# jmackey-astro/PION

Measured on AMD Instinct MI355X. Metric: Mcell-updates/s on 3D ideal-MHD 512³ uniform grid; achieved HBM GB/s vs peak, higher is better.
Workload: dtype f64; 1 GPU; M1: 3-D GLM-MHD (nvar 9) Stone blast wave 512^3, HLLD + FKJ98 eta 0.1, periodic, OA2/OA2; nvar=9, decomposition=z-slab x1, transport=none; time loop and transport issued from C++ (libpion_host), fp_mode=fast (FMA contraction)

## Files before the change

pion_amd/csrc/kernels.h:

```cpp
#ifndef PION_KERNELS_H
#define PION_KERNELS_H

#include <hip/hip_runtime.h>
#include <stdint.h>

#include "dev_riemann.h"
#include "grid_desc.h"
#include "rows_tiling.h"
#include "hll_screen.h"

namespace pion {

#define PION_MAX_NTR 2
#define PION_COOL_NT_MAX 256

struct CoolDev {
  int NT;
  const double *T;
  const double *tab;
  const double *slope;
  double inv_Mu2, inv_Mu2_elec_H, Mu_tot_over_kB;
  double MinT_allowed, MaxT_allowed;
  float lg0, inv_dlg;
};
// ... 27 lines not shown
  static constexpr int lds = 11 * PION_COOL_NT_MAX;
};

struct StageArgs {
  GridDesc g;
  const double *S;
  const double *Pc;
  double *out;
  const uint8_t *flags;
  const uint8_t *hllflag;
  const double *eta;
  int *errword;
  FluxCtx fc;
  int eqntype, ntracer, solver;
  int space_ooa;
  int cooling;
  double dt;
  double glm_damp;
  double max_temp;
  int use_march;
  int xwrap;
  int zslope_lds;
  double *dE;
  int zchunk;
  int nzb, zcmax;
  int rows;
  int rows_auto;
  int ncu;
  int kz0, kz1;
  int kz2, kz3;
  unsigned long long *dtres;
  double cfl;
  int dt_mp;
  int plain_cells;
  CoolDev cool;
  unsigned long long *hsum;
  long hsum_n;
  int hsum_nbx, hsum_nby, hsum_nbz;
};

struct PrepassArgs {
  GridDesc g;
  const double *S;
  uint8_t *hllflag;
  double *divv, *gradp;
  double *eta;
  int eqntype, nvar, space_ooa;
  double gamma;
  long c0, c1;
  long c2, c3;
  const unsigned long long *hsum;
  ScrGeom scr;
  int *scr_list, *scr_count;
};

struct DtArgs {
  GridDesc g;
  const double *P;
  const double *Ph;
  const uint8_t *flags;
  unsigned long long *result;
  int *errword;
  int eqntype, nvar;
  double gamma, cfl;
  int do_mp;
  CoolDev cool;
};

struct FluxTestArgs {
  int n, axis, eqntype, ntracer, solver;
  const double *Pl, *Pr, *aux;
  double *F, *Pstar;
  int *errword;
  FluxCtx fc;
};

struct CellTestArgs {
  int n, eqntype, ntracer;
  const double *Pin, *dU;
  double *Pout, *dt;
  StageArgs st;
};

struct CoolTestArgs {
  int n, nvar;
  double dt, gamma;
  const double *Pin;
  double *Pout;
  const double *rho, *T;
  double *edot;
  int *errword;
  CoolDev cool;
};

#define PION_PER_EQN(FN, ARGS, ...)                                            \
  int FN##_hd(const ARGS &a, __VA_OPT__(__VA_ARGS__ x, ) hipStream_t s);       \
  int FN##_mhd(const ARGS &a, __VA_OPT__(__VA_ARGS__ x, ) hipStream_t s);      \
  int FN##_glm(const ARGS &a, __VA_OPT__(__VA_ARGS__ x, ) hipStream_t s);      \
  inline int FN(const ARGS &a, __VA_OPT__(__VA_ARGS__ x, ) hipStream_t s)      \
  {                                                                            \
    if (a.eqntype == EQEUL) return FN##_hd(a, __VA_OPT__(x, ) s);              \
    if (a.eqntype == EQMHD) return FN##_mhd(a, __VA_OPT__(x, ) s);             \
    if (a.eqntype == EQGLM) return FN##_glm(a, __VA_OPT__(x, ) s);             \
    return -1;                                                                 \
  }

#define PION_DECLARE_FP(NS)                                        \
// ... 18 lines not shown
```

pion_amd/csrc/kernels_prepass.hip:

```cpp
#include "dev_cooling.h"
#include "kernels.h"

#ifndef PION_FPNS
#error "PION_FPNS must be defined (fp_strict or fp_fast)"
#endif

namespace pion {
namespace PION_FPNS {

#include "dev_sweep.h"

PDEV void prepass_hlld_cell(const PrepassArgs &a, const int *i);

__global__ __launch_bounds__(256) void k_prepass_hlld(const PrepassArgs a)
{
  const long nc = a.g.ncell;
  const unsigned gx = (a.g.nga[0] + 63) / 64, gy = (a.g.nga[1] + 3) / 4;
  const long plane = (long)a.g.nga[0] * a.g.nga[1];
  const unsigned npl1 = (unsigned)((a.c1 - a.c0) / plane);
  const unsigned npl = npl1 + ((a.c3 > a.c2) ? (unsigned)((a.c3 - a.c2) / plane) : 0u);
  const unsigned ntile = gx * gy * npl;
  const unsigned t = (unsigned)xcd_tile(blockIdx.x, ntile);
  if (t >= ntile) return;
  int i[3];
// ... 153 lines not shown
        if (s >= nvs) {
          eL[s] = eR[s] = 0.0;
          continue;
        }
        const double *b = a.S + (long)(mhd ? rotvar<true>(ax, s) : rotvar<false>(ax, s)) * nc + c;
        const double q0 = b[0], q1 = b[st];
        double s0 = 0.0, s1 = 0.0;
        if (oa2 && a.g.cyl == 2) {
          const double R0 = sph_R(a.g, k), R1 = sph_R(a.g, k + 1);
          const double c0 = sph_Rcom(R0, dx), c1 = sph_Rcom(R1, dx);
          if (k > 0) s0 = avg_falle((q0 - b[-st]) / (c0 - sph_Rcom(sph_R(a.g, k - 1), dx)), (q1 - q0) / (c1 - c0));
          if (k + 1 < n - 1) s1 = avg_falle((q1 - q0) / (c1 - c0), (b[2 * st] - q1) / (sph_Rcom(sph_R(a.g, k + 2), dx) - c1));
          eL[s] = q0 + s0 * (R0 + 0.5 * dx - c0);
          eR[s] = q1 + s1 * (R1 - 0.5 * dx - c1);
        }
        else if (oa2 && a.g.cyl == 1 && ax == 1) {
          const double R0 = cyl_R(a.g, k), R1 = cyl_R(a.g, k + 1);
          const double c0 = cyl_Rcom(R0, dx), c1 = cyl_Rcom(R1, dx);
          if (k > 0) s0 = avg_falle((q0 - b[-st]) / (c0 - cyl_Rcom(cyl_R(a.g, k - 1), dx)), (q1 - q0) / (c1 - c0));
          if (k + 1 < n - 1) s1 = avg_falle((q1 - q0) / (c1 - c0), (b[2 * st] - q1) / (cyl_Rcom(cyl_R(a.g, k + 2), dx) - c1));
          eL[s] = q0 + s0 * (R0 + dx * 0.5 - c0);
          eR[s] = q1 + s1 * (R1 - dx * 0.5 - c1);
        }
        else if (oa2) {
          if (k > 0) s0 = avg_falle((q0 - b[-st]) / dx, (q1 - q0) / dx);
          if (k + 1 < n - 1) s1 = avg_falle((q1 - q0) / dx, (b[2 * st] - q1) / dx);
          eL[s] = q0 + s0 * dx * 0.5;
          eR[s] = q1 - s1 * dx * 0.5;
        }
        else {
          eL[s] = q0;
          eR[s] = q1;
        }
      }
      double msL, msR;
      if (mhd) {
        msL = Eqn<EQMHD, 0>::cfast(eL, g);
        msR = Eqn<EQMHD, 0>::cfast(eR, g);
      }
      else {
        msL = Eqn<EQEUL, 0>::chydro(eL, g);
        msR = Eqn<EQEUL, 0>::chydro(eR, g);
      }
      eta = 0.5 * (fabs(eR[qVN] - eL[qVN]) + fabs(msR - msL));
    }
    a.eta[ax * nc + c] = eta;
  }
}

__global__ __launch_bounds__(256) void k_prepass_screen(const PrepassArgs a)
{
  const long nblk = scr_total(a.scr);
  const long t = (long)blockIdx.x * blockDim.x + threadIdx.x;
  if (t >= nblk) return;
  const int bx = (int)(t % a.scr.nb[0]), by = (int)((t / a.scr.nb[0]) % a.scr.nb[1]);
  const int bz = (int)(t / ((long)a.scr.nb[0] * a.scr.nb[1]));
  if (!scr_block_quiet(a.scr, a.hsum, a.hsum + nblk, bx, by, bz)) a.scr_list[atomicAdd(a.scr_count, 1)] = (int)t;
}
__global__ __launch_bounds__(256) void k_prepass_hlld_blocks(const PrepassArgs a)
{
  const int n = *a.scr_count;
  for (int e = (int)blockIdx.x; e < n; e += (int)gridDim.x) {
    const int t = a.scr_list[e];
    const int bx = t % a.scr.nb[0], by = (t / a.scr.nb[0]) % a.scr.nb[1], bz = t / (a.scr.nb[0] * a.scr.nb[1]);
    int lo[3], hi[3];
    scr_cells_ext(a.scr, 0, bx, &lo[0], &hi[0]);
    scr_cells_ext(a.scr, 1, by, &lo[1], &hi[1]);
    scr_cells_ext(a.scr, 2, bz, &lo[2], &hi[2]);
    const int ny = hi[1] - lo[1], nrow = ny * (hi[2] - lo[2]);
    for (int r = (int)(threadIdx.x >> 6); r < nrow; r += 4) {
      int i[3];
      i[1] = lo[1] + r % ny;
      i[2] = lo[2] + r / ny;
      for (i[0] = lo[0] + (int)(threadIdx.x & 63); i[0] < hi[0]; i[0] += 64) prepass_hlld_cell(a, i);
    }
  }
}

int launch_prepass(const PrepassArgs &a, hipStream_t s)
{
  const unsigned nb = (unsigned)((a.c1 - a.c0 + 255) / 256);
  if (a.hllflag && a.hsum) {
    const long nblk = scr_total(a.scr);
    if (hipMemsetAsync(a.hllflag, 0, (size_t)a.g.ncell, s) != hipSuccess) return -1;
    if (hipMemsetAsync(a.scr_count, 0, sizeof(int), s) != hipSuccess) return -1;
    hipLaunchKernelGGL(k_prepass_screen, dim3((unsigned)((nblk + 255) / 256)), dim3(256), 0, s, a);
    const unsigned ngrid = (nblk < 4096) ? (unsigned)nblk : 4096u;
    hipLaunchKernelGGL(k_prepass_hlld_blocks, dim3(ngrid), dim3(256), 0, s, a);
  }
  else if (a.hllflag) {
    const long plane = (long)a.g.nga[0] * a.g.nga[1];
    const unsigned npl = (unsigned)((a.c1 - a.c0) / plane) + ((a.c3 > a.c2) ? (unsigned)((a.c3 - a.c2) / plane) : 0u);
    const unsigned ntile = (unsigned)((a.g.nga[0] + 63) / 64) * ((a.g.nga[1] + 3) / 4) * npl;
    if (a.g.ndim == 2 && (a.c0 != 0 || a.c1 != a.g.ncell)) {
      const long row = a.g.nga[0];
      const unsigned nr = (unsigned)((a.c1 - a.c0) / row) + ((a.c3 > a.c2) ? (unsigned)((a.c3 - a.c2) / row) : 0u);
      if (nr > 0)
        hipLaunchKernelGGL(k_prepass_hlld_rows, dim3((unsigned)((a.g.nga[0] + 63) / 64) * ((nr + 3) / 4)), dim3(256), 0,
                           s, a);
    }
    else if (a.g.ndim == 3 && a.g.cyl == 0 && !a.divv && !a.gradp && a.c3 <= a.c2 && npl >= PION_PREPASS_ZC
        && a.g.ncell * 8L < (1L << 32)) {
      const unsigned nch = (npl + PION_PREPASS_ZC - 1) / PION_PREPASS_ZC;
      const unsigned nt = (unsigned)((a.g.nga[0] + 61) / 62) * ((a.g.nga[1] + 3) / 4) * nch;
      hipLaunchKernelGGL(k_prepass_hlld_march, dim3(((nt + 7) / 8) * 8), dim3(256), 0, s, a);
    }
    else hipLaunchKernelGGL(k_prepass_hlld, dim3(((ntile + 7) / 8) * 8), dim3(256), 0, s, a);
  }
  if (a.eta) hipLaunchKernelGGL((k_prepass_hcorr<8>), dim3(nb), dim3(256), 0, s, a);
  return (int)hipGetLastError();
}

}
}
```

pion_amd/csrc/pion_gpu.hip:

```cpp
#include <hip/hip_runtime.h>

#include <cmath>
#include <cstdio>
#include <cstdlib>
#include <cstring>

#include "pion_handle.h"

using namespace pion;
using namespace pion::impl;

int impl::order_after_unpack(Handle *h)
{
  if (h->comm_stream && h->comm_stream != h->stream && h->ev_unpacked_valid) {
    HCHECK(h, hipStreamWaitEvent(h->stream, h->ev_unpacked, 0));
    h->ev_unpacked_valid = false;
  }
  return 0;
}

long impl::cell_id(const GridDesc &g, int ix, int iy, int iz)
{
  return (long)(ix + g.nbc[0]) + g.sy * (iy + g.nbc[1]) + g.sz * (iz + g.nbc[2]);
}
// ... 179 lines not shown
    if (hipDeviceGetAttribute(&ncu, hipDeviceAttributeMultiprocessorCount, device) == hipSuccess) h->ncu = ncu;
  }
  GridDesc &g = h->g;
  g.ndim = cfg->ndim;
  g.ncell = 1;
  for (int a = 0; a < 3; a++) {
    g.ng[a] = (a < cfg->ndim) ? cfg->ng[a] : 1;
    g.nbc[a] = (a < cfg->ndim) ? cfg->nbc : 0;
    g.nga[a] = g.ng[a] + 2 * g.nbc[a];
    g.ncell *= g.nga[a];
    g.xmin[a] = cfg->xmin[a];
  }
  g.sy = g.nga[0];
  g.sz = (long)g.nga[0] * g.nga[1];
  g.dx = cfg->dx;
  g.cyl = (cfg->coord_sys == 2) ? 1 : ((cfg->coord_sys == 3) ? 2 : 0);
  g.sph_vol = nullptr;
  *handle = h;
  const bool rows3d = (g.ndim == 3 && g.nbc[2] >= 2);
  bool rows2d = (g.ndim == 2 && g.cyl != 2 && g.nbc[1] >= 2 && g.nbc[0] >= 2);
  if (const char *e = getenv("PION_ROWS_2D")) rows2d = rows2d && (atoi(e) != 0);
  bool windows = true;
  if (const char *e = getenv("PION_ROWS_WINDOWS")) windows = (atoi(e) != 0);
  if (const char *e = getenv("PION_ROWS_WINDOW_CELLS")) {
    const long v = atol(e);
    if (windows && v >= 1 && v <= PION_ROWS_WINDOW_CELLS) h->win_cells = v;
  }
  if (rows3d || rows2d) {
    const int sa = g.ndim - 1;
    h->win_whole = windows ? rows_windows_count(0, g.ng[sa], (sa == 2) ? g.sz : g.sy, g.nbc[sa], h->win_cells)
                           : (g.ncell < PION_ROWS_WINDOW_CELLS ? 1 : 0);
  }
  if (h->win_whole < 1) h->use_march = 0;
  if (h->use_march == 0) h->win_whole = 0;

  const size_t nb = sizeof(double) * (size_t)cfg->nvar * g.ncell;
  HCHECK(h, hipMalloc(&h->dP, nb));
  HCHECK(h, hipMalloc(&h->dPh, nb));
  HCHECK(h, hipMemset(h->dP, 0, nb));
  HCHECK(h, hipMemset(h->dPh, 0, nb));
  HCHECK(h, hipMalloc(&h->dflags, g.ncell));
  if (g.cyl == 2) {
    std::vector<double> vol(g.nga[0]);
    for (int i = 0; i < g.nga[0]; i++) {
      double rc = g.xmin[0] + (2 * (i - g.nbc[0]) + 1) * (0.5 * g.dx);
      const double rp = rc + 0.5 * g.dx;
      const double rn = rp - g.dx;
      vol[i] = (pow(rp, 3.0) - pow(rn, 3.0)) / 3.0;
    }
    HCHECK(h, hipMalloc(&h->dsphvol, sizeof(double) * vol.size()));
    HCHECK(h, hipMemcpy(h->dsphvol, vol.data(), sizeof(double) * vol.size(), hipMemcpyHostToDevice));
    g.sph_vol = h->dsphvol;
  }
  HCHECK(h, hipMalloc(&h->derr, 64));
  HCHECK(h, hipMemset(h->derr, 0, 64));
  HCHECK(h, hipMalloc(&h->ddt, 2 * sizeof(unsigned long long)));
  HCHECK(h, hipMalloc(&h->ddt_init, 2 * sizeof(unsigned long long)));
  {
    const double init[2] = {1.e100, 1.0e99};
    HCHECK(h, hipMemcpy(h->ddt_init, init, sizeof init, hipMemcpyHostToDevice));
  }
  if (cfg->eqntype != PION_EQEUL && cfg->solver == PION_FLUX_RS_HLLD) {
    HCHECK(h, hipMalloc(&h->dhll, g.ncell));
    HCHECK(h, hipMemset(h->dhll, 0, g.ncell));
  }
  if (cfg->cooling != 0) {
    HCHECK(h, hipMalloc(&h->ddE, sizeof(double) * g.ncell));
    HCHECK(h, hipMemset(h->ddE, 0, sizeof(double) * g.ncell));
  }
  if (cfg->artvisc == PION_AV_HCORRECTION || cfg->artvisc == PION_AV_HCORR_FKJ98) {
    HCHECK(h, hipMalloc(&h->deta, sizeof(double) * cfg->ndim * g.ncell));
    HCHECK(h, hipMemset(h->deta, 0, sizeof(double) * cfg->ndim * g.ncell));
  }

  h->hflags.assign(g.ncell, 0);
  for (long c = 0; c < g.ncell; c++) {
    int i[3];
    i[0] = (int)(c % g.nga[0]) - g.nbc[0];
    i[1] = (int)((c / g.nga[0]) % g.nga[1]) - g.nbc[1];
    i[2] = (int)(c / g.sz) - g.nbc[2];
    bool on = true;
    bool all_periodic_offgrid = true;
    for (int a = 0; a < cfg->ndim; a++) {
      if (i[a] < 0) {
        on = false;
        if (cfg->bc_type[2 * a] != PION_BC_PERIODIC) all_periodic_offgrid = false;
      }
      else if (i[a] >= g.ng[a]) {
        on = false;
        if (cfg->bc_type[2 * a + 1] != PION_BC_PERIODIC) all_periodic_offgrid = false;
      }
    }
    uint8_t f = PION_CELL_ISLEAF | PION_CELL_TIMESTEP;
    if (on) f |= PION_CELL_ISGD | PION_CELL_ISDOMAIN;
    else {
      f |= PION_CELL_ISBD;
      (void)all_periodic_offgrid;
    }
    h->hflags[c] = f;
  }
  HCHECK(h, hipMemcpy(h->dflags, h->hflags.data(), g.ncell, hipMemcpyHostToDevice));

  const double m_p = 1.672621898e-24, kB = 1.38064852e-16;
  const double Mu = 1.40 * m_p, Mu_tot = 0.609 * m_p, Mu_elec = 1.167 * m_p, Mu_ion = 1.273 * m_p;
  h->Mu_tot_over_kB = Mu_tot / kB;
  memset(&h->cool, 0, sizeof h->cool);
  h->cool.inv_Mu2 = 1.0 / (Mu * Mu);
  h->cool.inv_Mu2_elec_H = 1.0 / (Mu_elec * Mu);
  h->cool.Mu_tot_over_kB = h->Mu_tot_over_kB;
  h->cool.MinT_allowed = cfg->min_temp;
  h->cool.MaxT_allowed = cfg->max_temp;
  if (h->cool.MinT_allowed < 1.0 || h->cool.MinT_allowed > 1.0e6) h->cool.MinT_allowed = 1.0;
// ... 12 lines not shown
    const double refvel = sqrt(cfg->gamma * cfg->refvec[1] / cfg->refvec[0]);
    h->refvec_avg[2] = h->refvec_avg[3] = h->refvec_avg[4] = 0.1 * refvel;
  }
  else {
    double *rv = h->refvec_avg;
    const double gam = cfg->gamma;
    auto cfast = [&](const double *p) {
      const double ch = sqrt(gam * p[1] / p[0]);
      const double t1 = ch * ch + (p[5] * p[5] + p[6] * p[6] + p[7] * p[7]) / p[0];
      double t2 = 4. * ch * ch * p[5] * p[5] / p[0];
      t2 = std::max(5.e-16, t1 * t1 - t2);
      return sqrt((t1 + sqrt(t2)) / 2.);
    };
    auto rotate_xy = [&](double *v, double theta) {
      const double ct = cos(theta), st = sin(theta);
      double a = v[2] * ct - v[3] * st, b = v[2] * st + v[3] * ct;
      v[2] = a;
      v[3] = b;
      a = v[5] * ct - v[6] * st;
      b = v[5] * st + v[6] * ct;
      v[5] = a;
      v[6] = b;
    };
    double angle = rv[6] * rv[6] + rv[5] * rv[5], refvel;
    if (angle > 10. * 5.e-16) {
      angle = M_PI / 2. - asin(rv[6] / sqrt(angle));
      if (rv[5] < 0) angle = -angle;
      rotate_xy(rv, angle);
      refvel = cfast(rv);
      rotate_xy(rv, -angle);
    }
    else refvel = cfast(rv);
    const double refB = sqrt(rv[5] * rv[5] + rv[6] * rv[6] + rv[7] * rv[7]);
    rv[2] = rv[3] = rv[4] = 0.1 * refvel;
    rv[5] = rv[6] = rv[7] = refB;
  }
  bc_init(h);
  return PION_GPU_OK;
}

void pion_gpu_destroy(void *handle)
{
  Handle *h = use(handle);
  if (!h) return;
  hipSetDevice(h->device);
  hipDeviceSynchronize();
  if (h->own_state) {
    hipFree(h->dP);
    hipFree(h->dPh);
  }
  hipFree(h->dflags);
  hipFree(h->dhll);
  hipFree(h->dsum);
  hipFree(h->dscr_list);
  hipFree(h->dscr_count);
  hipFree(h->ddE);
  hipFree(h->dfits_bad);
  if (h->bstream) hipStreamDestroy(h->bstream);
  if (h->ev_pre) hipEventDestroy(h->ev_pre);
  if (h->ev_bdone) hipEventDestroy(h->ev_bdone);
  if (h->hdt) hipHostFree(h->hdt);
  if (h->ev_dt) hipEventDestroy(h->ev_dt);
  hipFree(h->deta);
  hipFree(h->dsphvol);
  hipFree(h->derr);
  hipFree(h->ddt);
  hipFree(h->ddt_init);
  wind_free(h);
  rt_free(h);
  hipFree(h->djet_idx);
  hipFree(h->djet_state);
  hipFree(h->dcoolT);
  hipFree(h->dcooltab);
  hipFree(h->dcoolslope);
  hipFree(h->dcurve);
  for (int s = 0; s < 4; s++)
    for (hipEvent_t e : h->ev[s]) hipEventDestroy(e);
  if (h->ev_packed_src) hipEventDestroy(h->ev_packed_src);
  if (h->ev_unpacked) hipEventDestroy(h->ev_unpacked);
  delete h;
}

int pion_gpu_last_error(void *handle, char *buf, int len)
{
  Handle *h = use(handle);
  if (!h || !buf || len <= 0) return PION_GPU_EINVAL;
  snprintf(buf, len, "%s", h->err.c_str());
  return 0;
}

long pion_gpu_ncell_all(void *handle) { return ((Handle *)handle)->g.ncell; }
int pion_gpu_ng_all(void *handle, int axis) { return ((Handle *)handle)->g.nga[axis]; }

int pion_gpu_upload(void *handle, const double *P_soa)
{
  Handle *h = use(handle);
  h->xghost_fresh = nullptr;
  const size_t nb = sizeof(double) * (size_t)h->cfg.nvar * h->g.ncell;
  HCHECK(h, hipMemcpyAsync(h->dP, P_soa, nb, hipMemcpyHostToDevice, h->stream));
  HCHECK(h, hipMemcpyAsync(h->dPh, h->dP, nb, hipMemcpyDeviceToDevice, h->stream));
  HCHECK(h, hipStreamSynchronize(h->stream));
  h->ph_valid = false;
  state_changed(h);
  h->dt_requested = false;
  h->dt_mp_pending = false;
  return 0;
}

int pion_gpu_download(void *handle, int which, double *P_soa)
{
  Handle *h = use(handle);
  const size_t nb = sizeof(double) * (size_t)h->cfg.nvar * h->g.ncell;
  const double *src = (which == 1 && h->ph_valid) ? h->dPh : h->dP;
  if (int rc = order_after_unpack(h)) return rc;
  HCHECK(h, hipMemcpyAsync(P_soa, src, nb, hipMemcpyDeviceToHost, h->stream));
  HCHECK(h, hipStreamSynchronize(h->stream));
  return check_errword(h);
}
// ... 59 lines not shown
  return 0;
}
int pion_gpu_set_comm_stream(void *handle, void *stream)
{
  Handle *h = use(handle);
  h->comm_stream = (hipStream_t)stream;
  h->ev_unpacked_valid = false;
  return 0;
}
int pion_gpu_synchronize(void *handle)
{
  Handle *h = use(handle);
  HCHECK(h, hipStreamSynchronize(h->stream));
  if (h->comm_stream && h->comm_stream != h->stream) HCHECK(h, hipStreamSynchronize(h->comm_stream));
  if (h->bstream) HCHECK(h, hipStreamSynchronize(h->bstream));
  return 0;
}

int pion_gpu_get_flags(void *handle, unsigned char *out)
{
  Handle *h = use(handle);
  if (!h || !out) return PION_GPU_EINVAL;
  HCHECK(h, hipMemcpyAsync(out, h->dflags, h->g.ncell, hipMemcpyDeviceToHost, h->stream));
  HCHECK(h, hipStreamSynchronize(h->stream));
  return 0;
}

int pion_gpu_get_hll_switch(void *handle, unsigned char *out)
{
  Handle *h = use(handle);
  if (!h || !out || !h->dhll) return PION_GPU_EINVAL;
  HCHECK(h, hipMemcpyAsync(out, h->dhll, h->g.ncell, hipMemcpyDeviceToHost, h->stream));
  HCHECK(h, hipStreamSynchronize(h->stream));
  return 0;
}

int pion_gpu_get_hcorr_eta(void *handle, int axis, double *out)
{
  Handle *h = use(handle);
  if (!h || !out || !h->deta || axis < 0 || axis >= h->g.ndim) return PION_GPU_EINVAL;
  HCHECK(h, hipMemcpyAsync(out, h->deta + (size_t)axis * h->g.ncell, sizeof(double) * h->g.ncell, hipMemcpyDeviceToHost,
                           h->stream));
  HCHECK(h, hipStreamSynchronize(h->stream));
  return 0;
}

int pion_gpu_get_hll_screen_counts(void *handle, int *active, int *total)
{
  Handle *h = use(handle);
  if (!h || !active || !total) return PION_GPU_EINVAL;
  *active = -1;
  *total = 0;
  if (!h->last_prepass_screened) return 0;
  HCHECK(h, hipMemcpyAsync(active, h->dscr_count, sizeof(int), hipMemcpyDeviceToHost, h->stream));
  HCHECK(h, hipStreamSynchronize(h->stream));
  *total = (int)scr_total(h->scr);
  return 0;
}

int pion_gpu_set_cooling_tables(void *handle, int nT, const double *T, const double *tabs, const double *slopes)
{
  Handle *h = use(handle);
  state_changed(h);
  if (nT < 2 || nT > PION_COOL_NT_MAX) {
    h->err = "cooling tables: 2 <= nT <= 256 required";
    return PION_GPU_EINVAL;
  }
  hipFree(h->dcoolT);
  hipFree(h->dcooltab);
  hipFree(h->dcoolslope);
  HCHECK(h, hipMalloc(&h->dcoolT, sizeof(double) * nT));
  HCHECK(h, hipMalloc(&h->dcooltab, sizeof(double) * 5 * nT));
  HCHECK(h, hipMalloc(&h->dcoolslope, sizeof(double) * 5 * nT));
  HCHECK(h, hipMemcpy(h->dcoolT, T, sizeof(double) * nT, hipMemcpyHostToDevice));
  HCHECK(h, hipMemcpy(h->dcooltab, tabs, sizeof(double) * 5 * nT, hipMemcpyHostToDevice));
  HCHECK(h, hipMemcpy(h->dcoolslope, slopes, sizeof(double) * 5 * nT, hipMemcpyHostToDevice));
  h->cool.lg0 = 0.0f;
  h->cool.inv_dlg = 0.0f;
  if (T[0] > 0.0 && T[nT - 1] > T[0]) {
    const double l0 = log2(T[0]), inv = (nT - 1) / (log2(T[nT - 1]) - l0);
    bool ok = true;
    for (int i = 0; i < nT && ok; i++) {
      if (!(T[i] > 0.0) || (i > 0 && !(T[i] > T[i - 1]))) ok = false;
      else if (fabs((log2(T[i]) - l0) * inv - i) > 0.25) ok = false;
    }
    if (ok) {
      h->cool.lg0 = (float)l0;
      h->cool.inv_dlg = (float)inv;
    }
  }
  if (const char *e = getenv("PION_COOL_BISECT")) {
    if (atoi(e) != 0) h->cool.inv_dlg = 0.0f;
  }
  h->cool.NT = nT;
  h->cool.T = h->dcoolT;
  h->cool.tab = h->dcooltab;
  h->cool.slope = h->dcoolslope;
  h->have_tables = true;
  return 0;
}

int pion_gpu_set_cooling_curve(void *handle, int n, const double *logT, const double *logL, const double *c,
                               double min_slope, double max_slope)
{
  Handle *h = use(handle);
  if (!h) return PION_GPU_EINVAL;
  state_changed(h);
// ... 236 lines not shown
```

pion_amd/csrc/pion_handle.h:

```cpp
#ifndef PION_HANDLE_H
#define PION_HANDLE_H

#include <string>
#include <vector>

#include "../../include/pion_gpu.h"
#include "kernels.h"
#include "wind_host.h"

namespace pion::impl {

struct Handle {
  pion_gpu_config cfg;
  GridDesc g;
  int device = 0;
  int ncu = 0;
  hipStream_t stream = 0;
  hipStream_t comm_stream = 0;
  hipEvent_t ev_packed_src = nullptr, ev_unpacked = nullptr;
  hipStream_t bstream = 0;
  hipEvent_t ev_pre = nullptr, ev_bdone = nullptr;
  bool ev_pre_valid = false;
  bool concurrent_strips = true;
  bool ev_unpacked_valid = false;
  double *dP = nullptr, *dPh = nullptr;
  bool own_state = true;
  uint8_t *dflags = nullptr, *dhll = nullptr;
  double *deta = nullptr;
  double *dsphvol = nullptr;
  int *derr = nullptr;
  unsigned long long *ddt = nullptr;
  unsigned long long *ddt_init = nullptr;
  double *hdt = nullptr;
  hipEvent_t ev_dt = nullptr;
  bool dt_requested = false;
  std::vector<uint8_t> hflags;
  double refval[6][PION_MAX_NVAR];
  int dmr2_cols = 0;
  long nwind = 0;
  long njet = 0;
  long *djet_idx = nullptr;
  double *djet_state = nullptr;
  long *dwind_idx = nullptr;
  double *dwind_state = nullptr;
  std::vector<WindSource> wsrc;
  long nws = 0;
  long *dws_idx = nullptr;
  double *dws_dist = nullptr, *dws_off = nullptr, *dws_state = nullptr;
  double *dws_theta = nullptr;
  bool have_angle = false;
  AngleTables angle;
  CoolDev cool;
  double *dcoolT = nullptr, *dcooltab = nullptr, *dcoolslope = nullptr;
  bool have_tables = false;
  CoolForm form;
  double *dcurve = nullptr;
  bool have_curve = false;
  double glm_chyp = 0.0, glm_cr = 0.0;
  double refvec_avg[PION_MAX_NVAR];
  bool ph_valid = false;
  bool dt_cached = false;
  std::string err;
  bool timing = false;
  std::vector<hipEvent_t> ev[4];
  double Mu_tot_over_kB = 0.0;
  int use_march = 3, zchunk = 0, rows = 0;
  int rows1 = 0;
  long win_cells = PION_ROWS_WINDOW_CELLS;
  int win_whole = 0;
  int launches_last_part = 0;
  const double *xghost_fresh = nullptr;
  int zslope_lds = 1;
  double *ddE = nullptr;
  bool fuse_dt = true;
  bool uneven_chunks = true;
  bool dt_mp_pending = false;
  bool split_dt_mp = true;
  bool fuse_bc = true;
  bool hll_screen = true;
  bool screen_ok = false;
  ScrGeom scr;
  unsigned long long *dsum = nullptr;
  int *dscr_list = nullptr, *dscr_count = nullptr;
  const double *sum_arr = nullptr;
  bool sum_bc = false;
  bool last_prepass_screened = false;
  unsigned long long *dfits_bad = nullptr;
  struct RtState *rt = nullptr;
};

static inline void state_changed(Handle *h)
{
  h->dt_cached = false;
  h->sum_arr = nullptr;
  h->sum_bc = false;
}

#define HCHECK(h, call)                                                            \
  do {                                                                             \
    hipError_t e_ = (call);                                                        \
    if (e_ != hipSuccess) {                                                        \
      (h)->err = std::string(#call) + ": " + hipGetErrorString(e_);                \
      return PION_GPU_EDEVICE;                                                     \
    }                                                                              \
  } while (0)

static inline Handle *use(void *handle)
{
  Handle *h = (Handle *)handle;
  if (h) (void)hipSetDevice(h->device);
  return h;
}

int order_after_unpack(Handle *h);
long cell_id(const GridDesc &g, int ix, int iy, int iz);
void time_begin(Handle *h, int slot);
inline void time_end(Handle *h, int slot) { time_begin(h, slot); }
FluxCtx make_fluxctx(const Handle *h, double fv_dt);
int check_errword(Handle *h);
struct StageStep { double dt; int space_ooa, is_full_step; };
void stage_physics(const Handle *h, const StageStep &st, StageArgs &a);

template <class F, class... A>
int fp_launch(Handle *h, int slot, const char *failed, F *strict, F *fast, const A &... a)
{
  time_begin(h, slot);
  const int rc = h->cfg.strict_fp ? strict(a...) : fast(a...);
  time_end(h, slot);
  if (rc != 0) h->err = failed;
  return (rc != 0) ? PION_GPU_EDEVICE : 0;
}

static inline bool mp_dt_limited(const pion_gpu_config &cfg)
{
  return cfg.cooling != 0 && cfg.mp_timestep_limit >= 1 && cfg.mp_timestep_limit <= 3;
}

static inline bool cool_is_form(const pion_gpu_config &cfg)
{
  return cfg.cooling != 0 && cfg.cooling != PION_COOL_WSS09_CIE_LINE_HEAT_COOL;
}
static inline const char *cool_missing(const Handle *h)
{
  const int f = h->cfg.cooling;
  if (f == PION_COOL_WSS09_CIE_LINE_HEAT_COOL && !h->have_tables) return "cooling tables not set";
  if (f >= PION_COOL_SD93_CIE && f <= PION_COOL_WSS09_CIE_ONLY_COOLING && !h->have_curve) return "cooling curve not set";
  return nullptr;
}
// ... 18 lines not shown
```

pion_amd/csrc/pion_step.hip:

```cpp
#include <algorithm>
#include <cmath>
#include <cstring>

#include "pion_handle.h"

using namespace pion;
using namespace pion::impl;

void impl::stage_physics(const Handle *h, const StageStep &st, StageArgs &a)
{
  const pion_gpu_config &cfg = h->cfg;
  a.g = h->g;
  a.flags = h->dflags;
  a.hllflag = h->dhll;
  a.eta = h->deta;
  a.errword = h->derr;
  a.fc = make_fluxctx(h, st.dt);
  a.eqntype = cfg.eqntype;
  a.ntracer = cfg.ntracer;
  a.solver = cfg.solver;
  a.space_ooa = st.space_ooa;
  a.cooling = cfg.cooling;
  a.dt = st.dt;
  a.glm_damp = exp(-st.dt * h->glm_chyp * h->glm_cr);
// ... 33 lines not shown
{
  DtArgs a;
  a.g = h->g;
  a.P = h->dP;
  a.Ph = Ph;
  a.flags = h->dflags;
  a.result = h->ddt;
  a.errword = h->derr;
  a.eqntype = h->cfg.eqntype;
  a.nvar = h->cfg.nvar;
  a.gamma = h->cfg.gamma;
  a.cfl = h->cfg.cfl;
  a.do_mp = do_mp;
  a.cool = h->cool;
  return a;
}


static inline int slab_axis(const Handle *h) { return h->g.ndim - 1; }
static bool stage_can_split(const Handle *h)
{
  const int sa = slab_axis(h);
  return h->use_march != 0 && !h->deta && (h->g.ndim == 3 || h->g.ndim == 2)
         && h->g.ng[sa] > 2 * h->g.nbc[sa] && !(h->cfg.tm_ooa == 1 && h->cfg.sp_ooa == 1);
}

static int launch_cooling_time(Handle *h, const DtArgs &d, hipStream_t s)
{
  return fp_launch(h, 3, "cooling-time kernel launch failed", fp_strict::launch_dt_mp, fp_fast::launch_dt_mp, d, h->form, s);
}

static bool screen_admitted(Handle *h)
{
  const pion_gpu_config &cfg = h->cfg;
  if (!h->hll_screen || !h->dhll || cfg.ndim != 3 || h->g.cyl != 0 || h->use_march == 0 || h->g.nbc[2] < 2) return false;
  if (any_wind(h) || h->njet > 0 || cfg.bc_dmach2) return false;
  if (h->g.ncell * 8L >= (1L << 32) || h->win_whole > 1) return false;
  int per[3];
  for (int d = 0; d < 3; d++) {
    for (int f = 2 * d; f < 2 * d + 2; f++) {
      const int t = cfg.bc_type[f];
      if (!(t == PION_BC_PERIODIC || t == PION_BC_OUTFLOW || t == PION_BC_ONEWAY_OUT || t == PION_BC_REFLECTING
            || t == PION_BC_AXISYMMETRIC))
        return false;
    }
    if ((cfg.bc_type[2 * d] == PION_BC_PERIODIC) != (cfg.bc_type[2 * d + 1] == PION_BC_PERIODIC)) return false;
    per[d] = (cfg.bc_type[2 * d] == PION_BC_PERIODIC) ? 1 : 0;
    if (!scr_axis_ok(h->g.ng[d], h->g.nbc[d])) return false;
  }
  h->scr = scr_geom(h->g.ng, h->g.nbc, per);
  if (!h->dsum) {
    const size_t n = (size_t)scr_total(h->scr);
    if (hipMalloc(&h->dsum, 2 * n * sizeof(unsigned long long)) != hipSuccess) return false;
    if (hipMalloc(&h->dscr_list, n * sizeof(int)) != hipSuccess) return false;
    if (hipMalloc(&h->dscr_count, sizeof(int)) != hipSuccess) return false;
    if (hipMemset(h->dscr_count, 0, sizeof(int)) != hipSuccess) return false;
  }
  return true;
}

struct Range {
  int lo = 0, hi = 0;
  bool empty() const { return hi <= lo; }
  int n() const { return empty() ? 0 : hi - lo; }
};

struct StagePart {
  Range r[2];
  bool first, last;
  hipStream_t stream;
  bool beside;
  bool whole() const { return first && last; }
};

int part_axis(const Handle *h) { return slab_axis(h) > 0 ? slab_axis(h) : 2; }
StagePart part_whole(const Handle *h) { return {{{0, h->g.ng[part_axis(h)]}, {}}, true, true, h->stream, false}; }
StagePart part_interior(const Handle *h)
{
  const int nz = h->g.ng[part_axis(h)], nb = h->g.nbc[part_axis(h)];
  return {{{nb, nz - nb}, {}}, true, false, h->stream, false};
}
StagePart part_strips(const Handle *h, hipStream_t side)
{
  const int nz = h->g.ng[part_axis(h)], nb = h->g.nbc[part_axis(h)];
  return {{{0, nb}, {nz - nb, nz}}, false, true, side ? side : h->stream, side != nullptr};
}

Range flag_planes(const StagePart &pt, const Range r, const int nb, const int nz)
{
  Range f = {r.lo - 1, r.hi + 1};
  if (!pt.first && f.lo < nb - 1) f.hi = std::min(f.hi, nb - 1);
  else if (!pt.first) f.lo = std::max(f.lo, nz - nb + 1);
  return r.empty() ? Range{} : Range{f.lo + nb, f.hi + nb};
}
void flag_cells(const Handle *h, const StagePart &pt, PrepassArgs &p)
{
  p.c1 = h->g.ncell;
  if (pt.whole()) return;
  const int sa = slab_axis(h), nb = h->g.nbc[sa], nz = h->g.ng[sa];
  const long sst = (sa == 2) ? h->g.sz : h->g.sy;
  const Range f0 = flag_planes(pt, pt.r[0], nb, nz), f1 = flag_planes(pt, pt.r[1], nb, nz);
  p.c0 = f0.lo * sst;
  p.c1 = f0.hi * sst;
  p.c2 = f1.lo * sst;
  p.c3 = f1.hi * sst;
}

int run_prepass(Handle *h, const StageStep &st, const StagePart &pt, const double *S)
{
  const pion_gpu_config &cfg = h->cfg;
  PrepassArgs p{};
  p.g = h->g;
  p.S = S;
  p.hllflag = h->dhll;
  p.eta = h->deta;
  p.eqntype = cfg.eqntype;
  p.nvar = cfg.nvar;
  p.space_ooa = st.space_ooa;
  p.gamma = cfg.gamma;
  flag_cells(h, pt, p);
  h->screen_ok = screen_admitted(h);
  if (pt.whole() && h->screen_ok && h->sum_arr == S && h->sum_bc) {
    p.hsum = h->dsum;
    p.scr = h->scr;
    p.scr_list = h->dscr_list;
    p.scr_count = h->dscr_count;
  }
  h->last_prepass_screened = (p.hsum != nullptr);
  return fp_launch(h, 1, "prepass launch failed", fp_strict::launch_prepass, fp_fast::launch_prepass, p, pt.stream);
}

int stage_arrays(Handle *h, const StageStep &st, const double *S, StageArgs &a)
{
  a.S = S;
  a.Pc = h->dP;
  a.out = st.is_full_step ? h->dP : h->dPh;
  if (st.is_full_step && !h->ph_valid && h->cfg.sp_ooa == 2 && st.space_ooa == 2) {
    h->err = "full-step stage requires a preceding half-step stage";
    return PION_GPU_EINVAL;
  }
  if (st.is_full_step && S == h->dP) a.out = h->dPh;
  return 0;
}

int stage_ranges(Handle *h, const StagePart &pt, StageArgs &a)
{
  const Range &r0 = pt.r[0], &r1 = pt.r[1];
  a.kz1 = 1;
  if (h->g.ndim == 3) {
    a.kz0 = r0.lo;
    a.kz1 = r0.hi;
    a.kz2 = r1.lo;
    a.kz3 = r1.empty() ? r1.lo : r1.hi;
  }
  else if (h->g.ndim == 2 && h->use_march != 0) {
    if (!r1.empty() && r1.n() != r0.n()) {
      h->err = "stage: the two row strips of a 2-D launch must have the same number of rows";
      return PION_GPU_EINVAL;
    }
    a.g.ng[1] = r0.n();
    a.kz0 = r0.lo;
    a.kz1 = r0.lo + 1;
    a.kz2 = r1.lo;
    a.kz3 = r1.empty() ? r1.lo : r1.lo + 1;
  }
  return 0;
}

void stage_tiling(const Handle *h, const int np, StageArgs &a)
{
  Rows2PlanIn p;
  p.ndim = h->g.ndim;
  p.nx = h->g.ng[0];
  p.ny = a.g.ng[1];
  p.np = (h->g.ndim == 3) ? np : 1;
  p.ncu = h->ncu;
  p.nv = h->cfg.nvar;
  p.euler = (h->cfg.eqntype == PION_EQEUL);
  p.march = (a.use_march != 0);
  p.zslope_lds = (a.zslope_lds != 0);
  p.second_order = (a.space_ooa == 2);
  p.uneven = h->uneven_chunks;
  p.want_rows = h->rows;
  p.want_rows1 = h->rows1;
  p.want_zchunk = h->zchunk;
  const Rows2Plan pl = rows2_plan(p);
  a.rows = pl.rows;
  a.rows_auto = pl.rows_auto;
  a.zchunk = pl.zchunk;
  a.zcmax = pl.zcmax;
  a.nzb = pl.nzb;
}

bool stage_windowed(const Handle *h) { return h->use_march != 0 && h->win_whole > 1 && h->g.ndim >= 2; }
StageArgs stage_window(const Handle *h, const StageArgs &part, const int w_lo, const int w_hi)
{
  StageArgs a = part;
  const long off = (long)w_lo * ((h->g.ndim == 3) ? h->g.sz : h->g.sy);
  a.S += off;
  a.Pc += off;
  a.out += off;
  a.flags += off;
  if (a.hllflag) a.hllflag += off;
  if (a.eta) a.eta += off;
  if (a.dE) a.dE += off;
  a.kz0 = a.kz2 = a.kz3 = 0;
  if (h->g.ndim == 3) a.kz1 = w_hi - w_lo;
  else {
    a.g.ng[1] = w_hi - w_lo;
    a.kz1 = 1;
    if (h->g.cyl == 1) a.g.xmin[1] = h->g.xmin[1] + w_lo * h->g.dx;
  }
  stage_tiling(h, w_hi - w_lo, a);
  return a;
}

struct StageExtras { bool fuse_dt, split_mp, leave_sum; };
int stage_extras(Handle *h, const StageStep &st, const StagePart &pt, StageArgs &a, StageExtras &x)
{
  const pion_gpu_config &cfg = h->cfg;
  x.fuse_dt = h->fuse_dt && st.is_full_step && st.space_ooa == 2 && a.use_march != 0
              && ((h->g.ndim == 3 && h->g.nbc[2] >= 2) || h->g.ndim == 2) && a.out == h->dP;
  x.split_mp = x.fuse_dt && mp_dt_limited(cfg) && (h->split_dt_mp || cool_is_form(cfg));
  x.leave_sum = pt.whole() && h->dhll && h->screen_ok && a.plain_cells && a.rows >= 1 && cfg.cooling == 0
                && !h->deta && !a.fc.mp.present
                && PION_SCR_BY % a.rows == 0 && !(st.is_full_step && a.out == h->dPh);
  state_changed(h);
  if (x.leave_sum) {
    a.hsum = h->dsum;
    a.hsum_n = scr_total(h->scr);
    a.hsum_nbx = h->scr.nb[0];
    a.hsum_nby = h->scr.nb[1];
    a.hsum_nbz = h->scr.nb[2];
    HCHECK(h, hipMemsetAsync(h->dsum, 0, 2 * (size_t)a.hsum_n * sizeof(unsigned long long), pt.stream));
  }
  a.dt_mp = (mp_dt_limited(cfg) && !x.split_mp) ? 1 : 0;
  if (x.fuse_dt) {
    if (pt.first)
      HCHECK(h, hipMemcpyAsync(h->ddt, h->ddt_init, 2 * sizeof(double), hipMemcpyDeviceToDevice, pt.stream));
    a.dtres = h->ddt;
  }
  return 0;
}

int stage_end(Handle *h, const StageStep &st, const StagePart &pt, const StageExtras &x, const StageArgs &a)
{
  if (x.split_mp) {
    if (pt.beside) h->dt_mp_pending = true;
    else if (int rc = launch_cooling_time(h, dt_args(h, h->dP, 1), pt.stream)) return rc;
  }
  if (st.is_full_step && a.out == h->dPh) {
    const size_t nb = sizeof(double) * (size_t)h->cfg.nvar * h->g.ncell;
    HCHECK(h, hipMemcpyAsync(h->dP, h->dPh, nb, hipMemcpyDeviceToDevice, pt.stream));
  }
  h->ph_valid = !st.is_full_step;
  h->dt_cached = x.fuse_dt;
  if (x.leave_sum) h->sum_arr = a.out;
  h->xghost_fresh = a.xwrap ? ((st.is_full_step && a.out == h->dPh) ? h->dP : a.out) : nullptr;
  return 0;
}

int stage_launch(Handle *h, const StageStep &st, const StagePart &pt)
{
  if (const char *m = cool_missing(h)) {
    h->err = m;
    return PION_GPU_EINVAL;
  }
  const double *S = h->ph_valid ? h->dPh : h->dP;
  if (int rc = (h->dhll || h->deta) ? run_prepass(h, st, pt, S) : 0) return rc;
  StageArgs a{};
  if (int rc = stage_arrays(h, st, S, a)) return rc;
  stage_physics(h, st, a);
  if (int rc = stage_ranges(h, pt, a)) return rc;
  stage_tiling(h, pt.r[0].n(), a);
  const bool form = cool_is_form(h->cfg);
  if (h->cfg.cooling != 0 && (form || a.use_march != 0)) {
    a.dE = h->ddE;
    StageArgs ac = a;
    if (a.use_march == 0) {
      ac.kz0 = 0;
      ac.kz1 = h->g.ng[2];
      ac.kz2 = ac.kz3 = 0;
    }
    if (int rc = fp_launch(h, 1, "cooling kernel launch failed", fp_strict::launch_cooling_dE, fp_fast::launch_cooling_dE,
                           ac, h->form, pt.stream))
      return rc;
  }
  StageExtras x;
  if (int rc = stage_extras(h, st, pt, a, x)) return rc;
  if (pt.first && !pt.last && h->concurrent_strips && !h->timing && h->comm_stream && h->comm_stream != h->stream) {
    if (!h->ev_pre) HCHECK(h, hipEventCreateWithFlags(&h->ev_pre, hipEventDisableTiming));
    HCHECK(h, hipEventRecord(h->ev_pre, pt.stream));
    h->ev_pre_valid = true;
  }
  const char *const failed = "stage kernel launch failed (unsupported eqn/solver/tracer combination?)";
  h->launches_last_part = 0;
  if (form && a.use_march == 0) {
    if (int rc = fp_launch(h, 0, failed, fp_strict::launch_stage_dE, fp_fast::launch_stage_dE, a, pt.stream)) return rc;
    h->launches_last_part = 1;
  }
  else if (!stage_windowed(h)) {
    if (int rc = fp_launch(h, 0, failed, fp_strict::launch_stage, fp_fast::launch_stage, a, pt.stream)) return rc;
    h->launches_last_part = 1;
  }
  else {
    const int sa = slab_axis(h);
    const long sst = (sa == 2) ? h->g.sz : h->g.sy;
    for (const Range &r : pt.r) {
      const int nw = rows_windows_count(r.lo, r.hi, sst, h->g.nbc[sa], h->win_cells);
      for (int i = 0; i < nw; i++) {
        int w_lo, w_hi;
        rows_window(r.lo, r.hi, nw, i, &w_lo, &w_hi);
        const StageArgs w = stage_window(h, a, w_lo, w_hi);
        if (int rc = fp_launch(h, 0, failed, fp_strict::launch_stage, fp_fast::launch_stage, w, pt.stream)) return rc;
        h->launches_last_part++;
      }
    }
  }
  return pt.last ? stage_end(h, st, pt, x, a) : 0;
}

hipStream_t halo_stream(const Handle *h) { return h->comm_stream ? h->comm_stream : h->stream; }
int halo_src_ready(Handle *h)
{
  if (halo_stream(h) == h->stream) return 0;
  if (!h->ev_packed_src) HCHECK(h, hipEventCreateWithFlags(&h->ev_packed_src, hipEventDisableTiming));
  HCHECK(h, hipEventRecord(h->ev_packed_src, h->stream));
  HCHECK(h, hipStreamWaitEvent(halo_stream(h), h->ev_packed_src, 0));
  return 0;
}
int halo_arrived(Handle *h)
{
  if (halo_stream(h) == h->stream) return 0;
  if (!h->ev_unpacked) HCHECK(h, hipEventCreateWithFlags(&h->ev_unpacked, hipEventDisableTiming));
  HCHECK(h, hipEventRecord(h->ev_unpacked, halo_stream(h)));
  h->ev_unpacked_valid = true;
  return 0;
}

}

extern "C" {

int pion_gpu_calc_dt_device(void *handle, void **dptr)
{
  Handle *h = use(handle);
  const DtArgs a = dt_args(h, h->ph_valid ? h->dPh : h->dP, mp_dt_limited(h->cfg) ? 1 : 0);
  if (const char *m = a.do_mp ? cool_missing(h) : nullptr) {
    h->err = m;
    return PION_GPU_EINVAL;
  }
  if (!h->dt_cached) {
    HCHECK(h, hipMemcpyAsync(h->ddt, h->ddt_init, 2 * sizeof(double), hipMemcpyDeviceToDevice, h->stream));
    const bool form = cool_is_form(h->cfg);
    DtArgs d = a;
    if (form) d.do_mp = 0;
    if (int rc = fp_launch(h, 3, "dt kernel launch failed", fp_strict::launch_dt, fp_fast::launch_dt, d, h->stream)) return rc;
    if (int rc = (form && a.do_mp) ? launch_cooling_time(h, a, h->stream) : 0) return rc;
    h->dt_cached = true;
  }
  if (dptr) *dptr = h->ddt;
  return 0;
}

int pion_gpu_dt_request(void *handle)
{
  Handle *h = use(handle);
  if (!h->hdt) HCHECK(h, hipHostMalloc((void **)&h->hdt, 4 * sizeof(double), hipHostMallocDefault));
  if (!h->ev_dt) HCHECK(h, hipEventCreateWithFlags(&h->ev_dt, hipEventDisableTiming));
  HCHECK(h, hipMemcpyAsync(h->hdt, h->ddt, 2 * sizeof(double), hipMemcpyDeviceToHost, h->stream));
  HCHECK(h, hipMemcpyAsync(h->hdt + 2, h->derr, sizeof(int), hipMemcpyDeviceToHost, h->stream));
  HCHECK(h, hipEventRecord(h->ev_dt, h->stream));
  h->dt_requested = true;
  return 0;
}

int pion_gpu_dt_wait(void *handle, double *t_dyn, double *t_mp)
{
  Handle *h = use(handle);
  if (!h->dt_requested) {
    h->err = "pion_gpu_dt_wait without pion_gpu_dt_request";
    return PION_GPU_EINVAL;
  }
  HCHECK(h, hipEventSynchronize(h->ev_dt));
  h->dt_requested = false;
  *t_dyn = h->hdt[0];
  *t_mp = h->hdt[1];
  int e;
  memcpy(&e, h->hdt + 2, sizeof e);
  if (e) return check_errword(h);
  return 0;
}

int pion_gpu_read_dt(void *handle, double *t_dyn, double *t_mp)
{
  if (int rc = pion_gpu_dt_request(handle)) return rc;
  return pion_gpu_dt_wait(handle, t_dyn, t_mp);
}

int pion_gpu_calc_dt(void *handle, double *t_dyn, double *t_mp)
{
  if (int rc = pion_gpu_calc_dt_device(handle, nullptr)) return rc;
  return pion_gpu_read_dt(handle, t_dyn, t_mp);
}

int pion_gpu_set_glm_speeds(void *handle, double dt, double dx, double cr)
{
  Handle *h = use(handle);
  h->glm_chyp = h->cfg.cfl * dx / dt;
  h->glm_cr = cr;
  return 0;
}

int pion_gpu_stage_part(void *handle, double dt_stage, int space_ooa, int is_full_step, int part)
{
  Handle *h = use(handle);
  const StageStep st = {dt_stage, space_ooa, is_full_step};
  if (part == PION_STAGE_WHOLE) {
    if (int rc = order_after_unpack(h)) return rc;
    return stage_launch(h, st, part_whole(h));
  }
  const bool split = stage_can_split(h);
  if (part == PION_STAGE_INTERIOR) {
    if (!split) return 0;
// ... 117 lines not shown
```

Before: 6317 Mcell-updates/s.

## Fold per-step memsets and copies into prepass kernels with sparse flag clearing

Removes the full-grid hllflag memset, the screen-count memset, the dsum memset and the dt-init copy each stage. Their work moves into the prepass screen and block kernels: previously active blocks that are now quiet get their flags cleared, and triple-buffered counters are reset on device. The dt and error words are merged so one device-to-host copy fetches both. It also splits each block's HLLD work into four z-quarters for more parallelism. This adds bookkeeping state (double-buffered lists, a call counter) that must stay consistent across state changes.

```diff
diff --git a/pion_amd/csrc/kernels.h b/pion_amd/csrc/kernels.h
--- a/pion_amd/csrc/kernels.h
+++ b/pion_amd/csrc/kernels.h
@@ -103,7 +103,15 @@
   const unsigned long long *hsum;
   ScrGeom scr;
   int *scr_list, *scr_count;
+  uint8_t *scr_now;
+  const int *scr_prev_list, *scr_prev_count;
+  int *scr_next_count;
+  unsigned long long *sum_clear;
+  unsigned long long *dt_reset;
 };
+
+#define PION_DT_INIT_DYN 1.e100
+#define PION_DT_INIT_MP 1.0e99
 
 struct DtArgs {
   GridDesc g;
diff --git a/pion_amd/csrc/kernels_prepass.hip b/pion_amd/csrc/kernels_prepass.hip
--- a/pion_amd/csrc/kernels_prepass.hip
+++ b/pion_amd/csrc/kernels_prepass.hip
@@ -229,28 +229,44 @@
 {
   const long nblk = scr_total(a.scr);
   const long t = (long)blockIdx.x * blockDim.x + threadIdx.x;
+  if (t == 0 && a.scr_next_count) *a.scr_next_count = 0;
   if (t >= nblk) return;
   const int bx = (int)(t % a.scr.nb[0]), by = (int)((t / a.scr.nb[0]) % a.scr.nb[1]);
   const int bz = (int)(t / ((long)a.scr.nb[0] * a.scr.nb[1]));
-  if (!scr_block_quiet(a.scr, a.hsum, a.hsum + nblk, bx, by, bz)) a.scr_list[atomicAdd(a.scr_count, 1)] = (int)t;
+  const bool quiet = scr_block_quiet(a.scr, a.hsum, a.hsum + nblk, bx, by, bz);
+  if (a.scr_now) a.scr_now[t] = quiet ? 0 : 1;
+  if (!quiet) a.scr_list[atomicAdd(a.scr_count, 1)] = (int)t;
 }
 __global__ __launch_bounds__(256) void k_prepass_hlld_blocks(const PrepassArgs a)
 {
   const int n = *a.scr_count;
-  for (int e = (int)blockIdx.x; e < n; e += (int)gridDim.x) {
-    const int t = a.scr_list[e];
+  const int nprev = a.scr_prev_list ? *a.scr_prev_count : 0;
+  for (long w = blockIdx.x; w < 4L * (nprev + n); w += gridDim.x) {
+    const int e = (int)(w >> 2), q = (int)(w & 3);
+    const bool clear = (e < nprev);
+    const int t = clear ? a.scr_prev_list[e] : a.scr_list[e - nprev];
+    if (clear && a.scr_now[t]) continue;
     const int bx = t % a.scr.nb[0], by = (t / a.scr.nb[0]) % a.scr.nb[1], bz = t / (a.scr.nb[0] * a.scr.nb[1]);
     int lo[3], hi[3];
     scr_cells_ext(a.scr, 0, bx, &lo[0], &hi[0]);
     scr_cells_ext(a.scr, 1, by, &lo[1], &hi[1]);
     scr_cells_ext(a.scr, 2, bz, &lo[2], &hi[2]);
-    const int ny = hi[1] - lo[1], nrow = ny * (hi[2] - lo[2]);
-    for (int r = (int)(threadIdx.x >> 6); r < nrow; r += 4) {
-      int i[3];
-      i[1] = lo[1] + r % ny;
-      i[2] = lo[2] + r / ny;
-      for (i[0] = lo[0] + (int)(threadIdx.x & 63); i[0] < hi[0]; i[0] += 64) prepass_hlld_cell(a, i);
-    }
+    const int zq = (hi[2] - lo[2] + 3) / 4, z0 = lo[2] + q * zq, z1 = (z0 + zq < hi[2]) ? z0 + zq : hi[2];
+    int i[3];
+    for (i[1] = lo[1] + (int)(threadIdx.x >> 6); i[1] < hi[1]; i[1] += 4)
+      for (i[2] = z0; i[2] < z1; i[2]++)
+        for (i[0] = lo[0] + (int)(threadIdx.x & 63); i[0] < hi[0]; i[0] += 64) {
+          if (clear) a.hllflag[(long)i[0] + a.g.sy * i[1] + a.g.sz * i[2]] = 0;
+          else prepass_hlld_cell(a, i);
+        }
+  }
+  if (a.sum_clear) {
+    const long ns = 2 * scr_total(a.scr);
+    for (long j = (long)blockIdx.x * blockDim.x + threadIdx.x; j < ns; j += (long)gridDim.x * blockDim.x) a.sum_clear[j] = 0;
+  }
+  if (a.dt_reset && blockIdx.x == 0 && threadIdx.x == 0) {
+    a.dt_reset[0] = (unsigned long long)__double_as_longlong(PION_DT_INIT_DYN);
+    a.dt_reset[1] = (unsigned long long)__double_as_longlong(PION_DT_INIT_MP);
   }
 }
 
@@ -259,8 +275,7 @@
   const unsigned nb = (unsigned)((a.c1 - a.c0 + 255) / 256);
   if (a.hllflag && a.hsum) {
     const long nblk = scr_total(a.scr);
-    if (hipMemsetAsync(a.hllflag, 0, (size_t)a.g.ncell, s) != hipSuccess) return -1;
-    if (hipMemsetAsync(a.scr_count, 0, sizeof(int), s) != hipSuccess) return -1;
+    if (!a.scr_prev_list && hipMemsetAsync(a.hllflag, 0, (size_t)a.g.ncell, s) != hipSuccess) return -1;
     hipLaunchKernelGGL(k_prepass_screen, dim3((unsigned)((nblk + 255) / 256)), dim3(256), 0, s, a);
     const unsigned ngrid = (nblk < 4096) ? (unsigned)nblk : 4096u;
     hipLaunchKernelGGL(k_prepass_hlld_blocks, dim3(ngrid), dim3(256), 0, s, a);
diff --git a/pion_amd/csrc/pion_gpu.hip b/pion_amd/csrc/pion_gpu.hip
--- a/pion_amd/csrc/pion_gpu.hip
+++ b/pion_amd/csrc/pion_gpu.hip
@@ -255,12 +255,12 @@
     HCHECK(h, hipMemcpy(h->dsphvol, vol.data(), sizeof(double) * vol.size(), hipMemcpyHostToDevice));
     g.sph_vol = h->dsphvol;
   }
-  HCHECK(h, hipMalloc(&h->derr, 64));
-  HCHECK(h, hipMemset(h->derr, 0, 64));
-  HCHECK(h, hipMalloc(&h->ddt, 2 * sizeof(unsigned long long)));
+  HCHECK(h, hipMalloc(&h->ddt, 4 * sizeof(unsigned long long)));
+  HCHECK(h, hipMemset(h->ddt, 0, 4 * sizeof(unsigned long long)));
+  h->derr = reinterpret_cast<int *>(h->ddt + 2);
   HCHECK(h, hipMalloc(&h->ddt_init, 2 * sizeof(unsigned long long)));
   {
-    const double init[2] = {1.e100, 1.0e99};
+    const double init[2] = {PION_DT_INIT_DYN, PION_DT_INIT_MP};
     HCHECK(h, hipMemcpy(h->ddt_init, init, sizeof init, hipMemcpyHostToDevice));
   }
   if (cfg->eqntype != PION_EQEUL && cfg->solver == PION_FLUX_RS_HLLD) {
@@ -379,8 +379,9 @@
   hipFree(h->dflags);
   hipFree(h->dhll);
   hipFree(h->dsum);
-  hipFree(h->dscr_list);
+  hipFree(h->dscr_list[0]);
   hipFree(h->dscr_count);
+  hipFree(h->dscr_now);
   hipFree(h->ddE);
   hipFree(h->dfits_bad);
   if (h->bstream) hipStreamDestroy(h->bstream);
@@ -390,7 +391,6 @@
   if (h->ev_dt) hipEventDestroy(h->ev_dt);
   hipFree(h->deta);
   hipFree(h->dsphvol);
-  hipFree(h->derr);
   hipFree(h->ddt);
   hipFree(h->ddt_init);
   wind_free(h);
@@ -556,7 +556,7 @@
   *active = -1;
   *total = 0;
   if (!h->last_prepass_screened) return 0;
-  HCHECK(h, hipMemcpyAsync(active, h->dscr_count, sizeof(int), hipMemcpyDeviceToHost, h->stream));
+  HCHECK(h, hipMemcpyAsync(active, h->dscr_count + (h->scr_calls - 1) % 3, sizeof(int), hipMemcpyDeviceToHost, h->stream));
   HCHECK(h, hipStreamSynchronize(h->stream));
   *total = (int)scr_total(h->scr);
   return 0;
diff --git a/pion_amd/csrc/pion_handle.h b/pion_amd/csrc/pion_handle.h
--- a/pion_amd/csrc/pion_handle.h
+++ b/pion_amd/csrc/pion_handle.h
@@ -28,8 +28,8 @@
   uint8_t *dflags = nullptr, *dhll = nullptr;
   double *deta = nullptr;
   double *dsphvol = nullptr;
+  unsigned long long *ddt = nullptr;
   int *derr = nullptr;
-  unsigned long long *ddt = nullptr;
   unsigned long long *ddt_init = nullptr;
   double *hdt = nullptr;
   hipEvent_t ev_dt = nullptr;
@@ -81,19 +81,28 @@
   bool screen_ok = false;
   ScrGeom scr;
   unsigned long long *dsum = nullptr;
-  int *dscr_list = nullptr, *dscr_count = nullptr;
   const double *sum_arr = nullptr;
   bool sum_bc = false;
   bool last_prepass_screened = false;
+  int *dscr_list[2] = {nullptr, nullptr}, *dscr_count = nullptr;
+  uint8_t *dscr_now = nullptr;
+  unsigned long long scr_calls = 0;
+  bool flags_sparse = false;
+  bool dsum_clean = false;
   unsigned long long *dfits_bad = nullptr;
   struct RtState *rt = nullptr;
 };
 
-static inline void state_changed(Handle *h)
+static inline void stage_result_dropped(Handle *h)
 {
   h->dt_cached = false;
   h->sum_arr = nullptr;
   h->sum_bc = false;
+}
+static inline void state_changed(Handle *h)
+{
+  stage_result_dropped(h);
+  h->flags_sparse = false;
 }
 
 #define HCHECK(h, call)                                                            \
diff --git a/pion_amd/csrc/pion_step.hip b/pion_amd/csrc/pion_step.hip
--- a/pion_amd/csrc/pion_step.hip
+++ b/pion_amd/csrc/pion_step.hip
@@ -109,9 +109,12 @@
   if (!h->dsum) {
     const size_t n = (size_t)scr_total(h->scr);
     if (hipMalloc(&h->dsum, 2 * n * sizeof(unsigned long long)) != hipSuccess) return false;
-    if (hipMalloc(&h->dscr_list, n * sizeof(int)) != hipSuccess) return false;
-    if (hipMalloc(&h->dscr_count, sizeof(int)) != hipSuccess) return false;
-    if (hipMemset(h->dscr_count, 0, sizeof(int)) != hipSuccess) return false;
+    if (hipMalloc(&h->dscr_list[0], 2 * n * sizeof(int)) != hipSuccess) return false;
+    h->dscr_list[1] = h->dscr_list[0] + n;
+    if (hipMalloc(&h->dscr_now, n) != hipSuccess) return false;
+    if (hipMalloc(&h->dscr_count, 3 * sizeof(int)) != hipSuccess) return false;
+    if (hipMemset(h->dscr_count, 0, 3 * sizeof(int)) != hipSuccess) return false;
+    h->dsum_clean = false;
   }
   return true;
 }
@@ -163,7 +166,7 @@
   p.c3 = f1.hi * sst;
 }
 
-int run_prepass(Handle *h, const StageStep &st, const StagePart &pt, const double *S)
+int run_prepass(Handle *h, const StageStep &st, const StagePart &pt, const double *S, const bool reset_dt, bool *did_reset_dt)
 {
   const pion_gpu_config &cfg = h->cfg;
   PrepassArgs p{};
@@ -180,11 +183,27 @@
   if (pt.whole() && h->screen_ok && h->sum_arr == S && h->sum_bc) {
     p.hsum = h->dsum;
     p.scr = h->scr;
-    p.scr_list = h->dscr_list;
-    p.scr_count = h->dscr_count;
+    const unsigned long long n = h->scr_calls;
+    p.scr_list = h->dscr_list[n & 1];
+    p.scr_count = h->dscr_count + n % 3;
+    p.scr_next_count = h->dscr_count + (n + 1) % 3;
+    p.scr_now = h->dscr_now;
+    if (h->flags_sparse && n > 0) {
+      p.scr_prev_list = h->dscr_list[(n - 1) & 1];
+      p.scr_prev_count = h->dscr_count + (n - 1) % 3;
+    }
+    p.sum_clear = h->dsum;
+    if (reset_dt) p.dt_reset = h->ddt;
   }
   h->last_prepass_screened = (p.hsum != nullptr);
-  return fp_launch(h, 1, "prepass launch failed", fp_strict::launch_prepass, fp_fast::launch_prepass, p, pt.stream);
+  *did_reset_dt = (p.dt_reset != nullptr);
+  const int rc = fp_launch(h, 1, "prepass launch failed", fp_strict::launch_prepass, fp_fast::launch_prepass, p, pt.stream);
+  h->flags_sparse = (rc == 0 && p.hllflag && p.hsum);
+  if (rc == 0 && p.hsum) {
+    h->scr_calls++;
+    h->dsum_clean = true;
+  }
+  return rc;
 }
 
 int stage_arrays(Handle *h, const StageStep &st, const double *S, StageArgs &a)
@@ -273,27 +292,33 @@
 }
 
 struct StageExtras { bool fuse_dt, split_mp, leave_sum; };
-int stage_extras(Handle *h, const StageStep &st, const StagePart &pt, StageArgs &a, StageExtras &x)
+bool stage_fuses_dt(const Handle *h, const StageStep &st, const StageArgs &a)
+{
+  return h->fuse_dt && st.is_full_step && st.space_ooa == 2 && a.use_march != 0
+         && ((h->g.ndim == 3 && h->g.nbc[2] >= 2) || h->g.ndim == 2) && a.out == h->dP;
+}
+int stage_extras(Handle *h, const StageStep &st, const StagePart &pt, const bool dt_is_reset, StageArgs &a, StageExtras &x)
 {
   const pion_gpu_config &cfg = h->cfg;
-  x.fuse_dt = h->fuse_dt && st.is_full_step && st.space_ooa == 2 && a.use_march != 0
-              && ((h->g.ndim == 3 && h->g.nbc[2] >= 2) || h->g.ndim == 2) && a.out == h->dP;
+  x.fuse_dt = stage_fuses_dt(h, st, a);
   x.split_mp = x.fuse_dt && mp_dt_limited(cfg) && (h->split_dt_mp || cool_is_form(cfg));
   x.leave_sum = pt.whole() && h->dhll && h->screen_ok && a.plain_cells && a.rows >= 1 && cfg.cooling == 0
                 && !h->deta && !a.fc.mp.present
                 && PION_SCR_BY % a.rows == 0 && !(st.is_full_step && a.out == h->dPh);
-  state_changed(h);
+  stage_result_dropped(h);
   if (x.leave_sum) {
     a.hsum = h->dsum;
     a.hsum_n = scr_total(h->scr);
     a.hsum_nbx = h->scr.nb[0];
     a.hsum_nby = h->scr.nb[1];
     a.hsum_nbz = h->scr.nb[2];
-    HCHECK(h, hipMemsetAsync(h->dsum, 0, 2 * (size_t)a.hsum_n * sizeof(unsigned long long), pt.stream));
+    if (!h->dsum_clean)
+      HCHECK(h, hipMemsetAsync(h->dsum, 0, 2 * (size_t)a.hsum_n * sizeof(unsigned long long), pt.stream));
+    h->dsum_clean = false;
   }
   a.dt_mp = (mp_dt_limited(cfg) && !x.split_mp) ? 1 : 0;
   if (x.fuse_dt) {
-    if (pt.first)
+    if (pt.first && !dt_is_reset)
       HCHECK(h, hipMemcpyAsync(h->ddt, h->ddt_init, 2 * sizeof(double), hipMemcpyDeviceToDevice, pt.stream));
     a.dtres = h->ddt;
   }
@@ -324,10 +349,12 @@
     return PION_GPU_EINVAL;
   }
   const double *S = h->ph_valid ? h->dPh : h->dP;
-  if (int rc = (h->dhll || h->deta) ? run_prepass(h, st, pt, S) : 0) return rc;
   StageArgs a{};
   if (int rc = stage_arrays(h, st, S, a)) return rc;
   stage_physics(h, st, a);
+  bool dt_is_reset = false;
+  if (int rc = (h->dhll || h->deta) ? run_prepass(h, st, pt, S, pt.first && stage_fuses_dt(h, st, a), &dt_is_reset) : 0)
+    return rc;
   if (int rc = stage_ranges(h, pt, a)) return rc;
   stage_tiling(h, pt.r[0].n(), a);
   const bool form = cool_is_form(h->cfg);
@@ -344,7 +371,7 @@
       return rc;
   }
   StageExtras x;
-  if (int rc = stage_extras(h, st, pt, a, x)) return rc;
+  if (int rc = stage_extras(h, st, pt, dt_is_reset, a, x)) return rc;
   if (pt.first && !pt.last && h->concurrent_strips && !h->timing && h->comm_stream && h->comm_stream != h->stream) {
     if (!h->ev_pre) HCHECK(h, hipEventCreateWithFlags(&h->ev_pre, hipEventDisableTiming));
     HCHECK(h, hipEventRecord(h->ev_pre, pt.stream));
@@ -425,8 +452,7 @@
   Handle *h = use(handle);
   if (!h->hdt) HCHECK(h, hipHostMalloc((void **)&h->hdt, 4 * sizeof(double), hipHostMallocDefault));
   if (!h->ev_dt) HCHECK(h, hipEventCreateWithFlags(&h->ev_dt, hipEventDisableTiming));
-  HCHECK(h, hipMemcpyAsync(h->hdt, h->ddt, 2 * sizeof(double), hipMemcpyDeviceToHost, h->stream));
-  HCHECK(h, hipMemcpyAsync(h->hdt + 2, h->derr, sizeof(int), hipMemcpyDeviceToHost, h->stream));
+  HCHECK(h, hipMemcpyAsync(h->hdt, h->ddt, 4 * sizeof(double), hipMemcpyDeviceToHost, h->stream));
   HCHECK(h, hipEventRecord(h->ev_dt, h->stream));
   h->dt_requested = true;
   return 0;
```

Result: no change. 6326 Mcell-updates/s, median of 2 (+0.1%).
